# brownvc/matryodshka

Measured on AMD Instinct MI355X. Metric: novel-view frames/sec, 640x320 ODS->32-sphere MSI infer+render, higher is better.
Workload: dtype f32

## Files before the change

matryodshka_amd/csrc/cnn.hip:

```cpp
#include "cnn_plan.h"

namespace msi_cnn {

int device_cu_count() {
  int dev = 0;
  hipDeviceProp_t prop;
  if (hipGetDevice(&dev) != hipSuccess || hipGetDeviceProperties(&prop, dev) != hipSuccess || prop.multiProcessorCount <= 0) {
    (void)hipGetLastError();
    return DEFAULT_CUS;
  }
  return prop.multiProcessorCount;
}

int launch_conv(const LayerLaunch &Q, const ConvParams &p, hipStream_t stream) {
  const ConvVariant &V = Q.variant;
  int rc;
  switch (V.family) {
    case CONV_IGEMM: rc = launch_igemm(Q, p, stream); break;
    case CONV_HALO: case CONV_HALO_S2: case CONVT_HALO: rc = launch_halo_f32(Q, p, stream); break;
    case CONV_HALO_X3: case CONV_HALO8_X3: case CONV_HALO_S2_X3: case CONV_HALO8_S2_X3: case CONVT_HALO_X3: case CONVT_HALO8_X3: rc = launch_x3(Q, p, stream); break;
    case CONV_HALO_BF16: case CONV_HALO_BF16_S2: case CONVT_HALO_BF16: rc = launch_bf16_halo(Q, p, stream); break;
    default: return msi::fail(MSI_E_UNSUPPORTED, "conv: unknown kernel family %d", V.family);
  }
  if (rc || Q.nfix == 0 || p.tile_cnt != nullptr) return rc;
  const int mode = V.family == CONV_IGEMM ? V.mode : (V.is_convt() ? MODE_CONVT : MODE_CONV);
  return launch_fixup(V.bm, V.bn, mode, V.family == CONV_IGEMM && V.bf16 && mode != MODE_HEAD, Q.nfix, V.is_convt() ? 2 : 1, p, stream);
}

}

#if defined(MSI_CONV_TIMING) || defined(MSI_DEBUG_STATS)
static unsigned long long *g_timing_buf = nullptr;
static int g_timing_layer = -1;
extern "C" int msi_debug_conv_occupancy(int lds_bytes) {
  return msi_cnn::debug_conv_occupancy(lds_bytes);
}
extern "C" void msi_debug_conv_timing(void *device_buffer, int layer) {
  g_timing_buf = static_cast<unsigned long long *>(device_buffer);
  g_timing_layer = layer;
}
#endif

extern "C" {

#ifdef MSI_DEBUG_SUMS
extern "C" long long msi_debug_sums_offset(const msi_net_plan *plan, int layer) { return (long long)plan->net.layers[layer].sums_off; }
extern "C" long long msi_debug_partial_offset(const msi_net_plan *plan) { return (long long)plan->net.partial_off; }
#endif
static int run_layers(const msi_net_plan *plan, const float *packed, const void *net_input, float *pred,
                      void *workspace, size_t workspace_bytes, msi_stream_t stream_, int nlayers) {
  MSI_REQUIRE(plan, "net_forward: null plan");
  const msi_net_desc *desc = &plan->desc;
  const Net &net = plan->net;
  const int bf16 = desc->dtype == MSI_DTYPE_BF16;
  MSI_REQUIRE(packed && net_input && workspace, "net_forward: null pointer");
  if (workspace_bytes < net.ws_bytes)
    return msi::fail(MSI_E_WORKSPACE, "net_forward: workspace %zu B < required %zu B", workspace_bytes,
                     net.ws_bytes);
  if (desc->batch == 0) return MSI_OK;
  hipStream_t stream = msi::as_stream(stream_);
  char *ws = static_cast<char *>(workspace);
  {
    const size_t n16 = net.zero_bytes / 16;
    int rc0 = launch_zero(ws + net.zero_off, n16, stream);
    if (rc0) return rc0;
  }
  int *cnt = reinterpret_cast<int *>(ws + net.cnt_off);
  for (int li = 0; li < nlayers; ++li) {
    const Layer &L = net.layers[li];
    const LayerLaunch &Q = plan->launch[li];
    ConvParams p = Q.p;
    auto src_ptr = [&](int s) -> const char * {
      if (s < 0) return static_cast<const char *>(net_input);
      return ws + (bf16 ? net.layers[s].act_off : net.layers[s].raw_off);
    };
    p.x0 = src_ptr(L.src0);
    p.x1 = L.src1 >= 0 ? src_ptr(L.src1) : p.x0;
    p.wpk = reinterpret_cast<const char *>(packed + L.packed_off);
    p.coord_bias = L.has_coord ? packed + L.coord_off : nullptr;
    p.bias = L.kind == MODE_HEAD ? packed + L.gamma_off : nullptr;
    if (Q.fuse_ln) {
      const Layer &S = net.layers[L.src0];
      p.ln_sums = reinterpret_cast<const long long *>(ws + S.sums_off);
      p.ln_gamma = packed + S.gamma_off;
      p.ln_beta = packed + S.beta_off;
    }
    p.y = L.kind == MODE_HEAD ? pred : reinterpret_cast<float *>(ws + L.raw_off);
    p.sums = L.kind == MODE_HEAD ? nullptr : reinterpret_cast<long long *>(ws + L.sums_off);
    auto scl_of = [&](int li2) { return reinterpret_cast<const double *>(packed + net.layers[li2].lnscl_off); };
    p.ln_scl = L.kind == MODE_HEAD ? nullptr : scl_of(li);
    p.ln_scl_src = L.src0 >= 0 ? scl_of(L.src0) : nullptr;
    p.ln_scl_src1 = L.src1 >= 0 ? scl_of(L.src1) : nullptr;
    p.status = reinterpret_cast<int *>(ws + net.err_off);
    p.partial = reinterpret_cast<float *>(ws + net.partial_off);
// ... 139 lines not shown
  const Net &net = plan->net;
  const Layer &H = net.layers[MSI_NET_NUM_LAYERS - 1];
  const int nd = desc->num_outputs / 2;
  const int bf16 = desc->dtype == MSI_DTYPE_BF16;
  if ((!bf16 && !plan->launch[MSI_NET_NUM_LAYERS - 1].fuse_ln) || (bf16 && !plan->opt[MSI_NET_OPT_HEAD_FUSE_LN]) ||
      H.c0 > 64 || H.c0 % 4 != 0 || desc->num_outputs != 2 * nd || nd % 4 != 0 || nd > 64 || desc->in_channels != 6 * nd ||
      ((long)desc->height * desc->width) % HA_TP != 0)
    return msi::fail(MSI_E_UNSUPPORTED, "%s: fused tail needs a blend_psv network (in = 6 D, out = 2 D, "
                     "D %% 4 == 0, D <= 64, ngf <= 64, HEAD_FUSE_LN on)", who);
  MSI_REQUIRE(rgba_native || layers_out, "%s: null pointer", who);
  MSI_REQUIRE(!layers_out || (reinterpret_cast<uintptr_t>(layers_out) & 15) == 0, "%s: layers_out is not 16-byte aligned", who);
  const int ng = (nd + HA_LG - 1) / HA_LG;
  if (nd % ng != 0 || (nd / ng) % 4 != 0 || (ng > 1 && bf16 && (nd / ng) % 8 != 0))
    return msi::fail(MSI_E_UNSUPPORTED, "%s: D = %d does not split into layer groups of a multiple of %d", who, nd, bf16 ? 8 : 4);
  int rc = run_layers(plan, packed, net_input, nullptr, workspace, workspace_bytes, stream_, MSI_NET_NUM_LAYERS - 1);
  if (rc || desc->batch == 0) return rc;
  hipStream_t stream = msi::as_stream(stream_);
  if (event_after_convs) {
    hipError_t e = hipEventRecord(static_cast<hipEvent_t>(event_after_convs), stream);
    if (e != hipSuccess) return msi::fail(MSI_E_LAUNCH, "%s: %s", who, hipGetErrorString(e));
  }
  char *ws = static_cast<char *>(workspace);
  const Layer &S = net.layers[H.src0];
  HeadAsmParams q;
  q.x = reinterpret_cast<const float *>(ws + S.raw_off);
  q.wpk = packed + H.packed_off;
  q.bias = packed + H.gamma_off;
  float *aff = reinterpret_cast<float *>(ws + S.aff_off);
  rc = launch_ln_finish(desc->batch, stream, reinterpret_cast<const long long *>(ws + S.sums_off), 1.0 / S.ln_count,
                        reinterpret_cast<const double *>(packed + S.lnscl_off), reinterpret_cast<int *>(ws + net.err_off),
                        packed + S.gamma_off, packed + S.beta_off, S.cout, aff, bf16);
  if (rc) return rc;
  q.aff = aff;
  q.psv = net_input;
  q.rgba = reinterpret_cast<float4 *>(rgba_native);
  q.layers = layers_out;
  q.bw_out = blend_weights;
  q.al_out = alphas;
  q.pred_out = pred;
  q.C0 = H.c0; q.ksteps = H.ksteps; q.npad = H.npad;
  q.nd = nd; q.hw = desc->height * desc->width;
  q.npix_total = (long)desc->batch * q.hw;
  q.lg = nd / ng;
  q.ng = ng;
  {
    auto magic = [](unsigned d) { return d == 1 ? 0xffffffffu : (unsigned)((1ull << 32) / d); };
    const int vec = bf16 ? 8 : 4;
    const unsigned vpp = (unsigned)((ng == 1 ? 6 * nd : 2 * 3 * q.lg) / vec);
    q.mg_vpp = magic(vpp);
    q.mg_nchunk = magic((unsigned)(q.ksteps * 8));
    q.mg_hw = magic((unsigned)q.hw);
    if (q.npix_total >= (1L << 32)) return msi::fail(MSI_E_UNSUPPORTED, "%s: more than 2^32 pixels per batch", who);
  }
  constexpr int BN = 64;
  size_t r_bytes = (size_t)q.ksteps * (HA_TP + BN) * ROW_BYTES;
  if (r_bytes < (size_t)HA_TP * (6 * q.lg + 1) * sizeof(float)) r_bytes = (size_t)HA_TP * (6 * q.lg + 1) * sizeof(float);
  if (bf16) {
    r_bytes = (size_t)q.ksteps * HA_TP * ROW_BYTES;
    if (r_bytes < (size_t)HA_TP * (3 * q.lg + 1) * sizeof(unsigned)) r_bytes = (size_t)HA_TP * (3 * q.lg + 1) * sizeof(unsigned);
  }
  const size_t lds = 2 * 64 * 4 + 64 + ((r_bytes + 15) & ~(size_t)15) + (size_t)HA_TP * (2 * q.lg + 1) * sizeof(float);
  const long ntile = q.npix_total / HA_TP;
  if (((ntile + 7) / 8) * 8 * ng >= (1L << 31)) return msi::fail(MSI_E_UNSUPPORTED, "%s: too many pixel tiles for one launch", who);
  return launch_head_assemble(bf16, layers_out ? format : MSI_LAYERS_F32, (unsigned)(((ntile + 7) / 8) * 8 * ng), lds, stream, q);
}

int msi_net_plan_forward_rgba(const msi_net_plan *plan, const float *packed, const void *net_input, float *rgba_native,
                              float *blend_weights, float *alphas, float *pred, void *workspace, size_t workspace_bytes,
                              msi_stream_t stream_, void *event_after_convs) {
  return forward_fused_tail("net_forward_rgba", plan, packed, net_input, rgba_native, nullptr, MSI_LAYERS_F32, blend_weights, alphas, pred,
                            workspace, workspace_bytes, stream_, event_after_convs);
}

int msi_net_plan_forward_layers(const msi_net_plan *plan, const float *packed, const void *net_input, float *rgba_native,
                                void *layers_out, int32_t format, float *blend_weights, float *alphas, float *pred, void *workspace,
                                size_t workspace_bytes, msi_stream_t stream_, void *event_after_convs) {
  MSI_REQUIRE(!layers_out || format == MSI_LAYERS_RGBA8 || format == MSI_LAYERS_RGBA16F,
              "net_forward_layers: unknown format %d (layers_out is MSI_LAYERS_RGBA8 or MSI_LAYERS_RGBA16F)", format);
  MSI_REQUIRE(rgba_native || layers_out, "net_forward_layers: null pointer");
  return forward_fused_tail("net_forward_layers", plan, packed, net_input, rgba_native, layers_out, format, blend_weights, alphas, pred,
                            workspace, workspace_bytes, stream_, event_after_convs);
}

size_t msi_net_workspace_bytes(const msi_net_desc *desc) {
  msi_net_plan *pl = nullptr;
  if (msi_net_plan_create(desc, &pl)) return 0;
  const size_t n = pl->net.ws_bytes;
  msi_net_plan_destroy(pl);
  return n;
}

static int forward_once(const msi_net_desc *desc, const float *packed, const void *net_input, float *pred,
                        void *workspace, size_t workspace_bytes, msi_stream_t stream) {
  msi_net_plan *pl = nullptr;
  int rc = msi_net_plan_create(desc, &pl);
  if (rc) return rc;
  rc = msi_net_plan_forward(pl, packed, net_input, pred, workspace, workspace_bytes, stream);
  msi_net_plan_destroy(pl);
  return rc;
}

int msi_net_forward_f32(const msi_net_desc *desc, const float *packed, const float *net_input,
                        float *pred, void *workspace, size_t workspace_bytes, msi_stream_t stream) {
  MSI_REQUIRE(desc && desc->dtype == MSI_DTYPE_F32, "net_forward_f32: desc->dtype must be MSI_DTYPE_F32");
  return forward_once(desc, packed, net_input, pred, workspace, workspace_bytes, stream);
}

int msi_net_forward_bf16(const msi_net_desc *desc, const float *packed, const void *net_input_bf16,
                         float *pred, void *workspace, size_t workspace_bytes, msi_stream_t stream) {
  MSI_REQUIRE(desc && desc->dtype == MSI_DTYPE_BF16, "net_forward_bf16: desc->dtype must be MSI_DTYPE_BF16");
  return forward_once(desc, packed, net_input_bf16, pred, workspace, workspace_bytes, stream);
}

}
```

matryodshka_amd/csrc/cnn_device.h:

```cpp
#pragma once
#include <cmath>
#include <cstdint>
#include <cstdio>
#include <cstdlib>
#include <cstring>
#include <new>
#include <type_traits>
#include <vector>

#include "msi_common.h"

namespace msi_cnn {


typedef float f32x16 __attribute__((ext_vector_type(16)));
typedef float v4f __attribute__((ext_vector_type(4)));
typedef __attribute__((address_space(3))) void lds_void;

constexpr int BK = 32;
constexpr int ROW_BYTES = BK * 4;
#ifndef MSI_NSTAGE
#define MSI_NSTAGE 2
#endif
constexpr int NSTAGE = MSI_NSTAGE;
// ... 67 lines not shown
  int apply;
  int planes;
  int waves;
  bool is_halo() const { return family != CONV_IGEMM; }
  bool is_convt_f32() const { return family == CONVT_HALO || family == CONVT_HALO_X3 || family == CONVT_HALO8_X3; }
  bool is_convt() const { return is_convt_f32() || family == CONVT_HALO_BF16; }
  bool six_product() const { return family >= CONV_HALO_X3 && family <= CONVT_HALO8_X3; }
  bool tile8() const { return family == CONV_HALO8_X3 || family == CONV_HALO8_S2_X3 || family == CONVT_HALO8_X3; }
};

struct LayerLaunch {
  ConvParams p;
  ConvVariant variant;
  int nblocks, nfix;
  int inlaunch;
  int fuse_ln;
  int skip_apply;
  unsigned ln_blocks;
};

constexpr int HA_TP = 32;
#ifndef MSI_HA_LG
#define MSI_HA_LG 32
#endif
constexpr int HA_LG = MSI_HA_LG;

struct HeadAsmParams {
  const float *x;
  const float *wpk;
  const float *bias;
  const float *aff;
  const void *psv;
  float4 *rgba;
  float *bw_out, *al_out;
  float *pred_out;
  int C0, ksteps, npad, nd, hw;
  int lg, ng;
  unsigned mg_vpp, mg_nchunk, mg_hw;
  long npix_total;
  void *layers;
};

int launch_conv(const LayerLaunch &Q, const ConvParams &p, hipStream_t stream);
int launch_igemm(const LayerLaunch &Q, const ConvParams &p, hipStream_t stream);
int launch_fixup(int bm, int bn, int mode, int raw16, unsigned grid_x, unsigned grid_y, const ConvParams &p, hipStream_t stream);
int launch_halo_f32(const LayerLaunch &Q, const ConvParams &p, hipStream_t stream);
int launch_x3(const LayerLaunch &Q, const ConvParams &p, hipStream_t stream);
int launch_bf16_halo(const LayerLaunch &Q, const ConvParams &p, hipStream_t stream);
int launch_zero(void *p, size_t n16, hipStream_t stream);
int launch_ln_finish(int batch, hipStream_t stream, const long long *sums, double inv_n, const double *scl, int *status, const float *gamma, const float *beta, int C,
                     float *aff, int raw16);
int launch_ln_apply(int bf16out, unsigned blocks, int batch, size_t lds, hipStream_t stream, float *x, const long long *sums, double inv_n, const double *scl, int *status,
                    const float *gamma, const float *beta, size_t per_sample, int C, float *aff, unsigned short *yb);
int launch_head_assemble(int bf16in, int format, unsigned grid_x, size_t lds, hipStream_t stream, const HeadAsmParams &q);
int debug_conv_occupancy(int lds_bytes);

constexpr int vkey(int family, int a = 0, int b = 0, int c = 0, int d = 0, int e = 0) { return ((((family * 16 + a) * 16 + b) * 16 + c) * 16 + d) * 16 + e; }

inline int set_max_lds(const void *fn, int lds, unsigned long long &done, const char *what) {
  int dev = 0;
  if (hipGetDevice(&dev) != hipSuccess) dev = 0;
  const bool tracked = dev >= 0 && dev < 64;
  if (tracked && ((done >> dev) & 1ull)) return MSI_OK;
  hipError_t e = hipFuncSetAttribute(fn, hipFuncAttributeMaxDynamicSharedMemorySize, lds);
  if (e != hipSuccess) return msi::fail(MSI_E_LAUNCH, "%s: %s", what, hipGetErrorString(e));
  if (tracked) done |= 1ull << dev;
  return MSI_OK;
}

template <auto KERNEL, int LDS, int THREADS = 256>
int launch_kernel(unsigned nblocks, const ConvParams &p, hipStream_t stream, const char *what) {
  if constexpr (LDS > 65536) {
    static thread_local unsigned long long done = 0;
    int rc0 = set_max_lds(reinterpret_cast<const void *>(KERNEL), LDS, done, what);
    if (rc0) return rc0;
  }
  hipLaunchKernelGGL(KERNEL, dim3(nblocks), dim3(THREADS), LDS, stream, p);
  return msi::check_launch(what);
}

template <int N> using IC = std::integral_constant<int, N>;
}
using namespace msi_cnn;

namespace {

template <int MODE>
__device__ __forceinline__ int tap_delta(int v, int parity, int rate, bool wrapt) {
  if (MODE == MODE_CONV) return v * rate;
  if (MODE == MODE_CONVT) return wrapt ? -v : (v == 0 ? 0 : (parity ? 1 : -1));
  return 0;
}

__device__ __forceinline__ unsigned udiv_magic(unsigned x, unsigned d, unsigned mg) {
  unsigned q = __umulhi(x, mg);
  if (x - q * d >= d) ++q;
  return q;
}

__device__ __forceinline__ int halo_row(const ConvParams &p, int tyi, int r, int rows_per_tile) {
  return p.row_par ? (tyi >> 1) * (2 * rows_per_tile) + (tyi & 1) + 2 * r : tyi * rows_per_tile + r;
}

__device__ __forceinline__ int xcd_contiguous(int bid, int n) {
  const int q = n >> 3, r = n & 7, xcd = bid & 7, local = bid >> 3;
  return (xcd < r ? xcd * (q + 1) : r * (q + 1) + (xcd - r) * q) + local;
}
// ... 618 lines not shown
```

matryodshka_amd/csrc/cnn_tail.hip:

```cpp
#include "cnn_device.h"

namespace {


template <int BF16IN>
__global__ void __launch_bounds__(256) __attribute__((amdgpu_waves_per_eu(BF16IN ? 6 : 5)))
head_assemble_kernel(const HeadAsmParams p) {
  [[maybe_unused]] constexpr int FMT = MSI_LAYERS_F32;
#include "cnn_tail_head_assemble.inc"
}

template <int BF16IN, int FMT>
__global__ void __launch_bounds__(256) __attribute__((amdgpu_waves_per_eu(BF16IN ? 6 : 5)))
head_assemble_packed_kernel(const HeadAsmParams p) {
  static_assert(FMT == MSI_LAYERS_RGBA8 || FMT == MSI_LAYERS_RGBA16F, "a packed texel format");
#include "cnn_tail_head_assemble.inc"
}

__global__ void __launch_bounds__(256)
ln_finish_kernel(const long long *__restrict__ sums, double inv_n, const double *__restrict__ scl, int *status,
                 const float *__restrict__ gamma, const float *__restrict__ beta, int C, float *__restrict__ aff, int raw16) {
  __shared__ double s_stat[2];
  const int b = blockIdx.x, tid = threadIdx.x;
  ln_mean_inv(sums + (size_t)b * LN_SHARDS * LN_WORDS, inv_n, scl, status, s_stat, tid);
  const double mu = s_stat[0], inv = s_stat[1];
  const double up = raw16 ? scl[2] * 16777216.0 : 1.0;
  for (int c = tid; c < C; c += 256) {
    const double sc = inv * (double)gamma[c];
    aff[(size_t)b * 2 * C + c] = (float)(sc * up);
    aff[(size_t)b * 2 * C + C + c] = (float)((double)beta[c] - mu * sc);
  }
}

__global__ void __launch_bounds__(256) zero_kernel(float4 *__restrict__ p, size_t n16) {
  const size_t i = (size_t)blockIdx.x * 256 + threadIdx.x;
  if (i < n16) p[i] = float4{0.f, 0.f, 0.f, 0.f};
}

template <int BF16OUT>
__global__ void __launch_bounds__(256)
ln_apply_kernel(float *__restrict__ x, const long long *__restrict__ sums, double inv_n, const double *__restrict__ scl,
                int *status, const float *__restrict__ gamma, const float *__restrict__ beta, size_t per_sample, int C,
                float *__restrict__ aff, unsigned short *__restrict__ yb) {
  extern __shared__ __attribute__((aligned(16))) float s_aff[];
  __shared__ double s_stat[2];
  const int b = blockIdx.y, tid = threadIdx.x;
  ln_mean_inv(sums + (size_t)b * LN_SHARDS * LN_WORDS, inv_n, scl, (blockIdx.x == 0 ? status : nullptr), s_stat, tid);
  const double mu = s_stat[0], inv = s_stat[1];
  const double up = BF16OUT ? scl[2] * 16777216.0 : 1.0;
  for (int c = tid; c < C; c += 256) {
    const double sc = inv * (double)gamma[c];
    const float fs = (float)sc, ft = (float)((double)beta[c] - mu * sc);
    s_aff[c] = BF16OUT ? (float)(sc * up) : fs;
    s_aff[C + c] = ft;
    if (blockIdx.x == 0) {
      aff[(size_t)b * 2 * C + c] = fs;
      aff[(size_t)b * 2 * C + C + c] = ft;
    }
  }
  __syncthreads();

  typedef _Float16 h4_t __attribute__((ext_vector_type(4)));
  const h4_t *xh = reinterpret_cast<const h4_t *>(reinterpret_cast<const _Float16 *>(x) + (size_t)b * per_sample);
  v4f *xv = reinterpret_cast<v4f *>(x + (size_t)b * per_sample);
  auto get = [&](size_t i) __attribute__((always_inline)) -> v4f {
    if (BF16OUT == 1) { const h4_t h = xh[i]; return v4f{(float)h.x, (float)h.y, (float)h.z, (float)h.w}; }
    return xv[i];
  };
  const size_t nvec = per_sample / 4;
  const size_t stride = (size_t)gridDim.x * blockDim.x;
  auto apply = [](v4f v, const v4f s4, const v4f t4) __attribute__((always_inline)) -> v4f {
    v.x = fmaxf(v.x * s4.x + t4.x, 0.f);
    v.y = fmaxf(v.y * s4.y + t4.y, 0.f);
    v.z = fmaxf(v.z * s4.z + t4.z, 0.f);
    v.w = fmaxf(v.w * s4.w + t4.w, 0.f);
    return v;
  };
  auto bf16_bits = [](float f) __attribute__((always_inline)) -> unsigned {
    const unsigned u = __builtin_bit_cast(unsigned, f);
    return (u + 0x7fffu + ((u >> 16) & 1u)) >> 16;
  };
  typedef unsigned v2u __attribute__((ext_vector_type(2)));
  v2u *yv = reinterpret_cast<v2u *>(yb + (size_t)b * per_sample);
  auto put = [&](size_t i, const v4f v) __attribute__((always_inline)) {
    if (BF16OUT == 1) yv[i] = v2u{bf16_bits(v.x) | (bf16_bits(v.y) << 16), bf16_bits(v.z) | (bf16_bits(v.w) << 16)};
    else xv[i] = v;
  };
  if ((256 * 4) % C == 0) {
    const int c = (tid * 4) % C;
    const v4f s4 = *reinterpret_cast<const v4f *>(s_aff + c);
    const v4f t4 = *reinterpret_cast<const v4f *>(s_aff + C + c);
    for (size_t i = (size_t)blockIdx.x * blockDim.x + tid; i < nvec; i += stride) put(i, apply(get(i), s4, t4));
  } else {
    for (size_t i = (size_t)blockIdx.x * blockDim.x + tid; i < nvec; i += stride) {
      const int c = (int)((i * 4) % C);
      put(i, apply(get(i), *reinterpret_cast<const v4f *>(s_aff + c), *reinterpret_cast<const v4f *>(s_aff + C + c)));
    }
  }
}

}

namespace msi_cnn {
int launch_zero(void *ptr, size_t n16, hipStream_t stream) {
  hipLaunchKernelGGL(zero_kernel, dim3((unsigned)((n16 + 255) / 256)), dim3(256), 0, stream, reinterpret_cast<float4 *>(ptr), n16);
  return msi::check_launch("zero");
}
int launch_ln_finish(int batch, hipStream_t stream, const long long *sums, double inv_n, const double *scl, int *status, const float *gamma, const float *beta, int C,
                     float *aff, int raw16) {
  hipLaunchKernelGGL(ln_finish_kernel, dim3(batch), dim3(256), 0, stream, sums, inv_n, scl, status, gamma, beta, C, aff, raw16);
  return msi::check_launch("ln_finish");
}
int launch_ln_apply(int bf16out, unsigned blocks, int batch, size_t lds, hipStream_t stream, float *x, const long long *sums, double inv_n, const double *scl, int *status,
                    const float *gamma, const float *beta, size_t per_sample, int C, float *aff, unsigned short *yb) {
  const dim3 grid(blocks, batch);
  if (bf16out) hipLaunchKernelGGL(ln_apply_kernel<1>, grid, dim3(256), lds, stream, x, sums, inv_n, scl, status, gamma, beta, per_sample, C, aff, yb);
  else hipLaunchKernelGGL(ln_apply_kernel<0>, grid, dim3(256), lds, stream, x, sums, inv_n, scl, status, gamma, beta, per_sample, C, aff, yb);
  return msi::check_launch("ln_apply");
}
int launch_head_assemble(int bf16in, int format, unsigned grid_x, size_t lds, hipStream_t stream, const HeadAsmParams &q) {
#define MSI_LAUNCH_HA(K) hipLaunchKernelGGL(K, dim3(grid_x), dim3(256), lds, stream, q)
  switch (format) {
    case MSI_LAYERS_F32:
      if (bf16in) MSI_LAUNCH_HA(head_assemble_kernel<1>); else MSI_LAUNCH_HA(head_assemble_kernel<0>);
      break;
    case MSI_LAYERS_RGBA8:
      if (bf16in) MSI_LAUNCH_HA((head_assemble_packed_kernel<1, MSI_LAYERS_RGBA8>)); else MSI_LAUNCH_HA((head_assemble_packed_kernel<0, MSI_LAYERS_RGBA8>));
      break;
    case MSI_LAYERS_RGBA16F:
      if (bf16in) MSI_LAUNCH_HA((head_assemble_packed_kernel<1, MSI_LAYERS_RGBA16F>)); else MSI_LAUNCH_HA((head_assemble_packed_kernel<0, MSI_LAYERS_RGBA16F>));
      break;
    default:
      return msi::fail(MSI_E_BADARG, "head_assemble: unknown format %d", format);
  }
#undef MSI_LAUNCH_HA
  return msi::check_launch("head_assemble");
}
}
```

matryodshka_amd/csrc/cnn_tail_head_assemble.inc:

```
#if defined(__HIP_DEVICE_COMPILE__)
  extern __shared__ __attribute__((aligned(16))) char smem[];
  constexpr int BN = 64;
  const int tid = threadIdx.x, lane = tid & 63, wave = tid >> 6;
  const int nd = p.nd, lg = p.lg, ng = p.ng;
  const unsigned slot = blockIdx.x >> 3;
  const unsigned tsl = ng == 1 ? slot : (ng == 2 ? slot >> 1 : slot / (unsigned)ng);
  const int g = (int)(slot - tsl * (unsigned)ng);
  const long tile = (long)tsl * 8 + (blockIdx.x & 7u);
  if (tile * HA_TP >= p.npix_total) return;
  const int c_psv = 6 * nd, c_pred = 2 * nd;
  const int l_cpsv = 6 * lg, l_cpred = 2 * lg;
  const int s_psv = l_cpsv + 1, s_pred = l_cpred + 1;
  const int s_psv16 = 3 * lg + 1;
  float *s_aff = reinterpret_cast<float *>(smem);
  char *sR = smem + 2 * 64 * 4 + 64;
  char *sA = sR;
  char *sB = sA + p.ksteps * HA_TP * ROW_BYTES;
  const size_t r_bytes = BF16IN ? max((size_t)p.ksteps * HA_TP * ROW_BYTES, (size_t)HA_TP * s_psv16 * sizeof(unsigned))
                                : max((size_t)p.ksteps * (HA_TP + BN) * ROW_BYTES, (size_t)HA_TP * s_psv * sizeof(float));
  float *l_psv = reinterpret_cast<float *>(sR);
  float *l_pred = reinterpret_cast<float *>(sR + ((r_bytes + 15) & ~(size_t)15));
  auto gcol = [&](int n) __attribute__((always_inline)) -> int { return n < lg ? g * lg + n : nd + g * lg + (n - lg); };

  const long p0 = tile * HA_TP;
  const int b = (int)udiv_magic((unsigned)p0, (unsigned)p.hw, p.mg_hw);
  constexpr int PSV_PER_THREAD = BF16IN ? 3 : 6;
  constexpr int B_PER_THREAD = 4;
  constexpr int PSV_VEC = BF16IN ? 8 : 4;
  constexpr int ESZ = BF16IN ? 2 : 4;
  const int nrun = ng == 1 ? 1 : 2;
  const int run_len = ng == 1 ? c_psv : 3 * lg;
  const int vpr = run_len / PSV_VEC, vpp = nrun * vpr;
  const int nv_psv = HA_TP * vpp;
  float4 q[PSV_PER_THREAD];
  {
    const char *gp = static_cast<const char *>(p.psv) + (size_t)p0 * c_psv * ESZ;
#pragma unroll
    for (int k = 0; k < PSV_PER_THREAD; ++k) {
      const int v = tid + 256 * k;
      if (v < nv_psv) {
        if (ng == 1) {
          q[k] = reinterpret_cast<const float4 *>(gp)[v];
        } else {
          const int px = (int)udiv_magic((unsigned)v, (unsigned)vpp, p.mg_vpp), w = v - px * vpp;
          const int r = w >= vpr ? 1 : 0, idx = w - r * vpr;
          const int start = r == 0 ? 3 * g * lg : 3 * (nd + g * lg);
          q[k] = *reinterpret_cast<const float4 *>(gp + ((size_t)px * c_psv + start + idx * PSV_VEC) * ESZ);
        }
      }
    }
  }
  const int nchunk = p.ksteps * 8;
  v4f araw[2];
  if (BF16IN) {
    typedef _Float16 h8_t __attribute__((ext_vector_type(8)));
    const int r = tid >> 3, c = (tid & 7) * 8;
    araw[0] = araw[1] = v4f{0.f, 0.f, 0.f, 0.f};
    if (c < p.C0) {
      const h8_t h = *reinterpret_cast<const h8_t *>(reinterpret_cast<const _Float16 *>(p.x) + (size_t)(p0 + r) * p.C0 + c);
      araw[0] = v4f{(float)h[0], (float)h[1], (float)h[2], (float)h[3]};
      araw[1] = v4f{(float)h[4], (float)h[5], (float)h[6], (float)h[7]};
    }
  } else {
#pragma unroll
    for (int k = 0; k < 2; ++k) {
      const int e = tid + 256 * k;
      const int r = (int)udiv_magic((unsigned)e, (unsigned)nchunk, p.mg_nchunk), c = (e - r * nchunk) * 4;
      araw[k] = v4f{0.f, 0.f, 0.f, 0.f};
      if (e < HA_TP * nchunk && c < p.C0) araw[k] = *reinterpret_cast<const v4f *>(p.x + (size_t)(p0 + r) * p.C0 + c);
    }
  }
  const int nb = p.ksteps * BN * 8;
  v4f braw[B_PER_THREAD];
  v4f wfrag[4];
  if (BF16IN) {
    if (wave < 2) {
      const int frow = lane & 31, fh = lane >> 5;
      const int nloc = wave * 32 + frow;
      const int gn = gcol(nloc < l_cpred ? nloc : 0);
      const int fswz = (gn >> 1) & 7;
#pragma unroll
      for (int qq = 0; qq < 4; ++qq) {
        wfrag[qq] = v4f{0.f, 0.f, 0.f, 0.f};
        if (nloc < l_cpred)
          wfrag[qq] = *reinterpret_cast<const v4f *>(p.wpk + (size_t)gn * (ROW_BYTES / 4) + (((2 * qq + fh) ^ fswz) << 2));
      }
    }
  } else {
#pragma unroll
    for (int k = 0; k < B_PER_THREAD; ++k) {
      const int e = tid + 256 * k;
      const int row = e >> 3, j = e & 7;
      const int ks = row / BN, n = row - ks * BN;
      braw[k] = v4f{0.f, 0.f, 0.f, 0.f};
      if (e < nb && n < l_cpred)
        braw[k] = *reinterpret_cast<const v4f *>(p.wpk + ((size_t)ks * p.npad + gcol(n)) * (ROW_BYTES / 4) + j * 4);
    }
  }
  if (tid < 2 * p.C0) s_aff[tid] = p.aff[(size_t)b * 2 * p.C0 + tid];
  __syncthreads();
  if (BF16IN) {
    const int r = tid >> 3, ch = tid & 7, c = ch * 8;
    unsigned pk[4] = {0u, 0u, 0u, 0u};
    if (c < p.C0) {
      float y[8];
#pragma unroll
      for (int k = 0; k < 2; ++k) {
        const v4f s4 = *reinterpret_cast<const v4f *>(s_aff + c + 4 * k), t4 = *reinterpret_cast<const v4f *>(s_aff + p.C0 + c + 4 * k);
        y[4 * k] = fmaxf(araw[k].x * s4.x + t4.x, 0.f); y[4 * k + 1] = fmaxf(araw[k].y * s4.y + t4.y, 0.f);
        y[4 * k + 2] = fmaxf(araw[k].z * s4.z + t4.z, 0.f); y[4 * k + 3] = fmaxf(araw[k].w * s4.w + t4.w, 0.f);
      }
#pragma unroll
      for (int k = 0; k < 4; ++k) asm("v_cvt_pk_bf16_f32 %0, %1, %2" : "=v"(pk[k]) : "v"(y[2 * k]), "v"(y[2 * k + 1]));
    }
    typedef unsigned v4u_t __attribute__((ext_vector_type(4)));
    *reinterpret_cast<v4u_t *>(sA + r * ROW_BYTES + ((ch ^ ((r >> 1) & 7)) << 4)) = v4u_t{pk[0], pk[1], pk[2], pk[3]};
  } else
#pragma unroll
  for (int k = 0; k < 2; ++k) {
    const int e = tid + 256 * k;
    if (e < HA_TP * nchunk) {
      const int r = (int)udiv_magic((unsigned)e, (unsigned)nchunk, p.mg_nchunk), ch = e - r * nchunk;
      const int c = ch * 4;
      v4f y = {0.f, 0.f, 0.f, 0.f};
      if (c < p.C0) {
        const v4f s4 = *reinterpret_cast<const v4f *>(s_aff + c), t4 = *reinterpret_cast<const v4f *>(s_aff + p.C0 + c);
        y.x = fmaxf(araw[k].x * s4.x + t4.x, 0.f); y.y = fmaxf(araw[k].y * s4.y + t4.y, 0.f);
        y.z = fmaxf(araw[k].z * s4.z + t4.z, 0.f); y.w = fmaxf(araw[k].w * s4.w + t4.w, 0.f);
      }
      const int ks = ch >> 3, chunk = ch & 7;
      *reinterpret_cast<v4f *>(sA + (ks * HA_TP + r) * ROW_BYTES + ((chunk ^ ((r >> 1) & 7)) << 4)) = y;
    }
  }
  if (!BF16IN) {
#pragma unroll
    for (int k = 0; k < B_PER_THREAD; ++k) {
      const int e = tid + 256 * k;
      if (e < nb) *reinterpret_cast<v4f *>(sB + (e >> 3) * ROW_BYTES + ((e & 7) << 4)) = braw[k];
    }
  }
  __syncthreads();
  if (wave < 2) {
    f32x16 acc;
#pragma unroll
    for (int r = 0; r < 16; ++r) acc[r] = 0.f;
    const int frow = lane & 31, fh = lane >> 5;
    const int fswz_a = (frow >> 1) & 7;
    const int fswz_b = (gcol(wave * 32 + frow < l_cpred ? wave * 32 + frow : 0) >> 1) & 7;
    if (BF16IN) {
      typedef __bf16 bf16x8 __attribute__((ext_vector_type(8)));
#pragma unroll
      for (int qq = 0; qq < 4; ++qq) {
        const v4f a = *reinterpret_cast<const v4f *>(sA + frow * ROW_BYTES + (((2 * qq + fh) ^ fswz_a) << 4));
        acc = __builtin_amdgcn_mfma_f32_32x32x16_bf16(__builtin_bit_cast(bf16x8, wfrag[qq]), __builtin_bit_cast(bf16x8, a), acc, 0, 0, 0);
      }
    } else
    for (int ks = 0; ks < p.ksteps; ++ks) {
#pragma unroll
      for (int qq = 0; qq < 4; ++qq) {
        const v4f a = *reinterpret_cast<const v4f *>(sA + (ks * HA_TP + frow) * ROW_BYTES + (((fh * 4 + qq) ^ fswz_a) << 4));
        const v4f w = *reinterpret_cast<const v4f *>(sB + (ks * BN + wave * 32 + frow) * ROW_BYTES + (((fh * 4 + qq) ^ fswz_b) << 4));
        acc = __builtin_amdgcn_mfma_f32_32x32x2f32(w.x, a.x, acc, 0, 0, 0);
        acc = __builtin_amdgcn_mfma_f32_32x32x2f32(w.y, a.y, acc, 0, 0, 0);
        acc = __builtin_amdgcn_mfma_f32_32x32x2f32(w.z, a.z, acc, 0, 0, 0);
        acc = __builtin_amdgcn_mfma_f32_32x32x2f32(w.w, a.w, acc, 0, 0, 0);
      }
    }
    const int px = lane & 31, half = lane >> 5;
#pragma unroll
    for (int gg = 0; gg < 4; ++gg) {
      const int n = wave * 32 + 8 * gg + 4 * half;
      if (n < l_cpred) {
        const int gn = gcol(n);
        const v4f bs = *reinterpret_cast<const v4f *>(p.bias + gn);
        v4f t = {msi_tanh(acc[4 * gg] + bs.x), msi_tanh(acc[4 * gg + 1] + bs.y), msi_tanh(acc[4 * gg + 2] + bs.z), msi_tanh(acc[4 * gg + 3] + bs.w)};
        if (p.pred_out) *reinterpret_cast<v4f *>(p.pred_out + (p0 + px) * c_pred + gn) = t;
        t.x = (t.x + 1.0f) / 2.0f; t.y = (t.y + 1.0f) / 2.0f; t.z = (t.z + 1.0f) / 2.0f; t.w = (t.w + 1.0f) / 2.0f;
        float *dst = l_pred + px * s_pred + n;
        dst[0] = t.x; dst[1] = t.y; dst[2] = t.z; dst[3] = t.w;
        if (n < lg) {
          if (p.bw_out) *reinterpret_cast<v4f *>(p.bw_out + (p0 + px) * nd + gn) = t;
        } else {
          if (p.al_out) *reinterpret_cast<v4f *>(p.al_out + (p0 + px) * nd + (gn - nd)) = t;
        }
      }
    }
  }
  __syncthreads();
#pragma unroll
  for (int k = 0; k < PSV_PER_THREAD; ++k) {
    const int v = tid + 256 * k;
    if (v < nv_psv) {
      const int px = (int)udiv_magic((unsigned)v, (unsigned)vpp, p.mg_vpp), w = v - px * vpp;
      if (BF16IN) {
        unsigned *dst = reinterpret_cast<unsigned *>(l_psv) + px * s_psv16 + w * 4;
        dst[0] = __builtin_bit_cast(unsigned, q[k].x); dst[1] = __builtin_bit_cast(unsigned, q[k].y);
        dst[2] = __builtin_bit_cast(unsigned, q[k].z); dst[3] = __builtin_bit_cast(unsigned, q[k].w);
      } else {
        float *dst = l_psv + px * s_psv + w * PSV_VEC;
        dst[0] = q[k].x; dst[1] = q[k].y; dst[2] = q[k].z; dst[3] = q[k].w;
      }
    }
  }
  __syncthreads();
  {
#pragma clang fp contract(off)
    const int px = tid & (HA_TP - 1);
    const long pp = p0 + px;
    const long off = pp - (long)b * p.hw;
    const float *rp = l_psv + px * s_psv;
    const float *rq = l_pred + px * s_pred;
    float4 *dst = p.rgba + ((long)b * nd + g * lg + tid / HA_TP) * p.hw + off;
    const long dstep = (long)(256 / HA_TP) * p.hw;
    constexpr int TEXEL_BYTES = FMT == MSI_LAYERS_RGBA8 ? 4 : 8;
    char *dstp = FMT != MSI_LAYERS_F32 ? static_cast<char *>(p.layers) + (((long)b * nd + g * lg + tid / HA_TP) * p.hw + off) * TEXEL_BYTES : nullptr;
    const bool want_f32 = FMT == MSI_LAYERS_F32 || p.rgba != nullptr;
    const unsigned *rp16 = reinterpret_cast<const unsigned *>(l_psv) + px * s_psv16;
    for (int d = tid / HA_TP; d < lg; d += 256 / HA_TP, dst += dstep, dstp += dstep * TEXEL_BYTES) {
      float fgv[3], bgv[3];
      if (BF16IN) {
        const int ef = 3 * d, eb = 3 * (lg + d);
        const unsigned f0 = rp16[ef >> 1], f1 = rp16[(ef >> 1) + 1], b0 = rp16[eb >> 1], b1 = rp16[(eb >> 1) + 1];
        const unsigned long long fw = ((unsigned long long)f1 << 32 | f0) >> ((ef & 1) * 16), bw = ((unsigned long long)b1 << 32 | b0) >> ((eb & 1) * 16);
#pragma unroll
        for (int c = 0; c < 3; ++c) {
          fgv[c] = __builtin_bit_cast(float, (unsigned)(fw >> (16 * c)) << 16);
          bgv[c] = __builtin_bit_cast(float, (unsigned)(bw >> (16 * c)) << 16);
        }
      } else {
#pragma unroll
        for (int c = 0; c < 3; ++c) { fgv[c] = rp[d * 3 + c]; bgv[c] = rp[(lg + d) * 3 + c]; }
      }
      const float *fg = fgv;
      const float *bg = bgv;
      const float w = rq[d];
      const float omw = 1.0f - w;
      float4 o;
      o.x = w * fg[0] + omw * bg[0];
      o.y = w * fg[1] + omw * bg[1];
      o.z = w * fg[2] + omw * bg[2];
      o.w = rq[lg + d];
      if constexpr (FMT == MSI_LAYERS_RGBA8) *reinterpret_cast<unsigned *>(dstp) = rgba8_encode(o);
      else if constexpr (FMT == MSI_LAYERS_RGBA16F) *reinterpret_cast<u32x2_g *>(dstp) = rgba16f_encode(o);
      if (want_f32) {
#if defined(MSI_HA_NT) && MSI_HA_NT
        __builtin_nontemporal_store(o.x, &dst->x); __builtin_nontemporal_store(o.y, &dst->y); __builtin_nontemporal_store(o.z, &dst->z); __builtin_nontemporal_store(o.w, &dst->w);
#else
        *dst = o;
#endif
      }
    }
  }
#endif
```

matryodshka_amd/isa_lint.py:

```python
import os
import re
import struct
import subprocess
import sys
import tempfile

def _find_objdump():
    import shutil
    cands = [os.environ.get("LLVM_OBJDUMP")]
    hipcc = os.environ.get("HIPCC") or shutil.which("hipcc") or "/opt/rocm/bin/hipcc"
    if hipcc and os.path.exists(hipcc):
        root = os.path.dirname(os.path.dirname(os.path.realpath(hipcc)))
        cands += [os.path.join(root, "lib", "llvm", "bin", "llvm-objdump"), os.path.join(root, "llvm", "bin", "llvm-objdump")]
    cands += [os.path.join(os.environ.get("ROCM_PATH", "/opt/rocm"), "lib", "llvm", "bin", "llvm-objdump"), "/opt/rocm/lib/llvm/bin/llvm-objdump",
              shutil.which("llvm-objdump")]
    for c in cands:
        if c and os.path.exists(c):
            return c
    raise RuntimeError("isa_lint: llvm-objdump not found (set LLVM_OBJDUMP)")


OBJDUMP = None
MAGIC = b"__CLANG_OFFLOAD_BUNDLE__"
FORBIDDEN = re.compile(r"^\s*(v_pk_(?:mul|add|fma)_f32|v_pk_mov_b32)\b.*\bop_sel:\[[01,]*1[01,]*\]")
# ... 16 lines not shown
        return None
    ops = [o.strip() for o in m.group(2).split(",")]
    data = ops[0] if "buffer" in m.group(1) else (ops[1] if len(ops) > 1 else "")
    return _vrange(data)


def _valu_dest(ins):
    t = ins.strip()
    if not t.startswith("v_") or t.startswith(NOT_A_VGPR_WRITE):
        return None
    parts = t.split(None, 1)
    if len(parts) < 2:
        return None
    return _vrange(parts[1].split(",")[0])


LOAD = re.compile(r"^(?:t?buffer_load_|global_load_|flat_load_|scratch_load_|ds_read|ds_load|ds_bpermute|ds_permute|ds_swizzle|ds_consume|ds_append|image_)")
DS_RETURN = re.compile(r"^ds_\w+_rtn_")
ATOMIC_RETURN = re.compile(r"^(?:buffer|global|flat)_atomic_")


def vgpr_writes(ins):
    t = ins.strip()
    parts = t.split(None, 1)
    if len(parts) < 2:
        return []
    mn, ops = parts[0], [o.strip() for o in parts[1].split(",")]
    out = []
    if mn.startswith("v_"):
        d = _valu_dest(t)
        if d is not None:
            out.append((d, "valu"))
        if mn.startswith("v_swap_b32") and len(ops) > 1 and _vrange(ops[1].split()[0]) is not None:
            out.append((_vrange(ops[1].split()[0]), "valu"))
    elif LOAD.match(mn) or DS_RETURN.match(mn):
        if re.search(r"\blds\b", parts[1]):
            return []
        d = _vrange(ops[0].split()[0]) if ops and ops[0] else None
        if d is not None:
            out.append((d, "load"))
    elif ATOMIC_RETURN.match(mn) and re.search(r"\b(?:glc|sc0)\b", parts[1]):
        d = _vrange(ops[0].split()[0]) if ops and ops[0] else None
        if d is not None:
            out.append((d, "load"))
    return out


def scan_kernel_text(lines):
    bad = []
    nstore = nload = 0
    pending = []
    for ins in lines:
        if not ins.strip():
            continue
        if pending:
            writes = vgpr_writes(ins)
            keep = []
            for p in pending:
                hit = [k for d, k in writes if not (d[1] < p[0][0] or d[0] > p[0][1])]
                if hit and "valu" not in hit:
                    nload += 1
                if "valu" in hit:
                    bad.append(p[1] + "  -> (%d wait state(s)) ->  " % p[2] + ins.strip())
                    continue
                mn = re.match(r"\s*s_nop\s+(\d+)", ins)
                p[2] += int(mn.group(1)) + 1 if mn else 1
                if p[2] < WIDE_STORE_WAIT_STATES:
                    keep.append(p)
            pending = keep
        sd = _store_data(ins)
        if sd is not None:
            nstore += 1
            pending.append([sd, ins.strip(), 0])
    return bad, nstore, nload


def _fatbin_section(path):
    data = open(path, "rb").read()
    assert data[:4] == b"\x7fELF" and data[4] == 2, "64-bit ELF expected"
    shoff, = struct.unpack_from("<Q", data, 0x28)
    shentsize, shnum, shstrndx = struct.unpack_from("<HHH", data, 0x3A)
    def sh(i):
        name, typ, flags, addr, off, size = struct.unpack_from("<IIQQQQ", data, shoff + i * shentsize)
        return name, off, size
    _, stroff, strsize = sh(shstrndx)
    for i in range(shnum):
        name, off, size = sh(i)
        end = data.index(b"\0", stroff + name)
        if data[stroff + name:end] == b".hip_fatbin":
            return data[off:off + size]
    raise RuntimeError("no .hip_fatbin section in " + path)


def code_objects(path):
    sec = _fatbin_section(path)
    out = []
    pos = sec.find(MAGIC)
    while pos >= 0:
        n, = struct.unpack_from("<Q", sec, pos + len(MAGIC))
        p = pos + len(MAGIC) + 8
        for _ in range(n):
            off, size, tlen = struct.unpack_from("<QQQ", sec, p)
            triple = sec[p + 24:p + 24 + tlen].decode()
            p += 24 + tlen
            if "amdgcn" in triple and size:
                out.append((triple, sec[pos + off:pos + off + size]))
# ... 50 lines not shown
```

Measured before the change: 539.2.

## Add direct head-assemble path reading sweep volume into registers, skipping LDS staging

Adds a DIRECT variant of the fused head-assemble kernel for the fp32 path. Each thread loads its pixel's foreground and background PSV colors straight from global memory into registers. It computes the blend in registers and writes the RGBA texels directly, so the LDS staging of the sweep volume and the B-operand LDS buffer go away. The MFMA uses fp32 32x32x2 on register weight fragments, and the second k-step's weights can be loaded late. The aim is smaller LDS use, which allows more waves per EU, plus fewer barriers. The cost is wider strided global reads and writes that coalesce less well, and a slower fp32 MFMA form.

```diff
diff --git a/matryodshka_amd/csrc/cnn.hip b/matryodshka_amd/csrc/cnn.hip
--- a/matryodshka_amd/csrc/cnn.hip
+++ b/matryodshka_amd/csrc/cnn.hip
@@ -1,4 +1,6 @@
 #include "cnn_plan.h"
+
+#include <atomic>
 
 namespace msi_cnn {
 
@@ -40,6 +42,10 @@
   g_timing_layer = layer;
 }
 #endif
+
+static std::atomic<int> g_tail_form{-1};
+static int tail_form_default(int out_format) { return out_format == MSI_LAYERS_F32 ? 0 : 1; }
+extern "C" int msi_debug_tail_form(int form) { return g_tail_form.exchange(form < 0 ? -1 : (form ? 1 : 0)); }
 
 extern "C" {
 
@@ -285,9 +291,13 @@
     q.mg_hw = magic((unsigned)q.hw);
     if (q.npix_total >= (1L << 32)) return msi::fail(MSI_E_UNSUPPORTED, "%s: more than 2^32 pixels per batch", who);
   }
+  const int out_format = layers_out ? format : MSI_LAYERS_F32;
+  const int forced = g_tail_form.load(std::memory_order_relaxed);
+  const int direct = bf16 ? 0 : (forced >= 0 ? forced : tail_form_default(out_format));
   constexpr int BN = 64;
   size_t r_bytes = (size_t)q.ksteps * (HA_TP + BN) * ROW_BYTES;
   if (r_bytes < (size_t)HA_TP * (6 * q.lg + 1) * sizeof(float)) r_bytes = (size_t)HA_TP * (6 * q.lg + 1) * sizeof(float);
+  if (direct) r_bytes = (size_t)q.ksteps * HA_TP * ROW_BYTES;
   if (bf16) {
     r_bytes = (size_t)q.ksteps * HA_TP * ROW_BYTES;
     if (r_bytes < (size_t)HA_TP * (3 * q.lg + 1) * sizeof(unsigned)) r_bytes = (size_t)HA_TP * (3 * q.lg + 1) * sizeof(unsigned);
@@ -295,7 +305,7 @@
   const size_t lds = 2 * 64 * 4 + 64 + ((r_bytes + 15) & ~(size_t)15) + (size_t)HA_TP * (2 * q.lg + 1) * sizeof(float);
   const long ntile = q.npix_total / HA_TP;
   if (((ntile + 7) / 8) * 8 * ng >= (1L << 31)) return msi::fail(MSI_E_UNSUPPORTED, "%s: too many pixel tiles for one launch", who);
-  return launch_head_assemble(bf16, layers_out ? format : MSI_LAYERS_F32, (unsigned)(((ntile + 7) / 8) * 8 * ng), lds, stream, q);
+  return launch_head_assemble(bf16, direct, out_format, (unsigned)(((ntile + 7) / 8) * 8 * ng), lds, stream, q);
 }
 
 int msi_net_plan_forward_rgba(const msi_net_plan *plan, const float *packed, const void *net_input, float *rgba_native,
diff --git a/matryodshka_amd/csrc/cnn_device.h b/matryodshka_amd/csrc/cnn_device.h
--- a/matryodshka_amd/csrc/cnn_device.h
+++ b/matryodshka_amd/csrc/cnn_device.h
@@ -143,7 +143,7 @@
                      float *aff, int raw16);
 int launch_ln_apply(int bf16out, unsigned blocks, int batch, size_t lds, hipStream_t stream, float *x, const long long *sums, double inv_n, const double *scl, int *status,
                     const float *gamma, const float *beta, size_t per_sample, int C, float *aff, unsigned short *yb);
-int launch_head_assemble(int bf16in, int format, unsigned grid_x, size_t lds, hipStream_t stream, const HeadAsmParams &q);
+int launch_head_assemble(int bf16in, int direct, int format, unsigned grid_x, size_t lds, hipStream_t stream, const HeadAsmParams &q);
 int debug_conv_occupancy(int lds_bytes);
 
 constexpr int vkey(int family, int a = 0, int b = 0, int c = 0, int d = 0, int e = 0) { return ((((family * 16 + a) * 16 + b) * 16 + c) * 16 + d) * 16 + e; }
diff --git a/matryodshka_amd/csrc/cnn_tail.hip b/matryodshka_amd/csrc/cnn_tail.hip
--- a/matryodshka_amd/csrc/cnn_tail.hip
+++ b/matryodshka_amd/csrc/cnn_tail.hip
@@ -1,4 +1,11 @@
 #include "cnn_device.h"
+
+#ifndef MSI_HA_DIRECT_WAVES
+#define MSI_HA_DIRECT_WAVES 6
+#endif
+#ifndef MSI_HA_DIRECT_WSPLIT
+#define MSI_HA_DIRECT_WSPLIT 1
+#endif
 
 namespace {
 
@@ -7,6 +14,7 @@
 __global__ void __launch_bounds__(256) __attribute__((amdgpu_waves_per_eu(BF16IN ? 6 : 5)))
 head_assemble_kernel(const HeadAsmParams p) {
   [[maybe_unused]] constexpr int FMT = MSI_LAYERS_F32;
+  [[maybe_unused]] constexpr bool DIRECT = false;
 #include "cnn_tail_head_assemble.inc"
 }
 
@@ -14,6 +22,23 @@
 __global__ void __launch_bounds__(256) __attribute__((amdgpu_waves_per_eu(BF16IN ? 6 : 5)))
 head_assemble_packed_kernel(const HeadAsmParams p) {
   static_assert(FMT == MSI_LAYERS_RGBA8 || FMT == MSI_LAYERS_RGBA16F, "a packed texel format");
+  [[maybe_unused]] constexpr bool DIRECT = false;
+#include "cnn_tail_head_assemble.inc"
+}
+
+__global__ void __launch_bounds__(256) __attribute__((amdgpu_waves_per_eu(MSI_HA_DIRECT_WAVES)))
+head_assemble_direct_kernel(const HeadAsmParams p) {
+  [[maybe_unused]] constexpr int BF16IN = 0, FMT = MSI_LAYERS_F32;
+  [[maybe_unused]] constexpr bool DIRECT = true;
+#include "cnn_tail_head_assemble.inc"
+}
+
+template <int FMT>
+__global__ void __launch_bounds__(256) __attribute__((amdgpu_waves_per_eu(MSI_HA_DIRECT_WAVES)))
+head_assemble_direct_packed_kernel(const HeadAsmParams p) {
+  static_assert(FMT == MSI_LAYERS_RGBA8 || FMT == MSI_LAYERS_RGBA16F, "a packed texel format");
+  [[maybe_unused]] constexpr int BF16IN = 0;
+  [[maybe_unused]] constexpr bool DIRECT = true;
 #include "cnn_tail_head_assemble.inc"
 }
 
@@ -118,8 +143,18 @@
   else hipLaunchKernelGGL(ln_apply_kernel<0>, grid, dim3(256), lds, stream, x, sums, inv_n, scl, status, gamma, beta, per_sample, C, aff, yb);
   return msi::check_launch("ln_apply");
 }
-int launch_head_assemble(int bf16in, int format, unsigned grid_x, size_t lds, hipStream_t stream, const HeadAsmParams &q) {
+int launch_head_assemble(int bf16in, int direct, int format, unsigned grid_x, size_t lds, hipStream_t stream, const HeadAsmParams &q) {
 #define MSI_LAUNCH_HA(K) hipLaunchKernelGGL(K, dim3(grid_x), dim3(256), lds, stream, q)
+  if (direct && bf16in) return msi::fail(MSI_E_UNSUPPORTED, "head_assemble: the direct form reads an fp32 sweep volume");
+  if (direct) {
+    switch (format) {
+      case MSI_LAYERS_F32: MSI_LAUNCH_HA(head_assemble_direct_kernel); break;
+      case MSI_LAYERS_RGBA8: MSI_LAUNCH_HA(head_assemble_direct_packed_kernel<MSI_LAYERS_RGBA8>); break;
+      case MSI_LAYERS_RGBA16F: MSI_LAUNCH_HA(head_assemble_direct_packed_kernel<MSI_LAYERS_RGBA16F>); break;
+      default: return msi::fail(MSI_E_BADARG, "head_assemble: unknown format %d", format);
+    }
+    return msi::check_launch("head_assemble");
+  }
   switch (format) {
     case MSI_LAYERS_F32:
       if (bf16in) MSI_LAUNCH_HA(head_assemble_kernel<1>); else MSI_LAUNCH_HA(head_assemble_kernel<0>);
diff --git a/matryodshka_amd/csrc/cnn_tail_head_assemble.inc b/matryodshka_amd/csrc/cnn_tail_head_assemble.inc
--- a/matryodshka_amd/csrc/cnn_tail_head_assemble.inc
+++ b/matryodshka_amd/csrc/cnn_tail_head_assemble.inc
@@ -12,11 +12,15 @@
   const int l_cpsv = 6 * lg, l_cpred = 2 * lg;
   const int s_psv = l_cpsv + 1, s_pred = l_cpred + 1;
   const int s_psv16 = 3 * lg + 1;
+  static_assert(!DIRECT || !BF16IN, "the direct form reads an fp32 sweep volume");
+  const int dpx = tid >> 3, dj = tid & 7;
+  const bool d_owns = 4 * dj < lg;
   float *s_aff = reinterpret_cast<float *>(smem);
   char *sR = smem + 2 * 64 * 4 + 64;
   char *sA = sR;
   char *sB = sA + p.ksteps * HA_TP * ROW_BYTES;
-  const size_t r_bytes = BF16IN ? max((size_t)p.ksteps * HA_TP * ROW_BYTES, (size_t)HA_TP * s_psv16 * sizeof(unsigned))
+  const size_t r_bytes = DIRECT ? (size_t)p.ksteps * HA_TP * ROW_BYTES
+                       : BF16IN ? max((size_t)p.ksteps * HA_TP * ROW_BYTES, (size_t)HA_TP * s_psv16 * sizeof(unsigned))
                                 : max((size_t)p.ksteps * (HA_TP + BN) * ROW_BYTES, (size_t)HA_TP * s_psv * sizeof(float));
   float *l_psv = reinterpret_cast<float *>(sR);
   float *l_pred = reinterpret_cast<float *>(sR + ((r_bytes + 15) & ~(size_t)15));
@@ -33,7 +37,14 @@
   const int vpr = run_len / PSV_VEC, vpp = nrun * vpr;
   const int nv_psv = HA_TP * vpp;
   float4 q[PSV_PER_THREAD];
-  {
+  if (DIRECT) {
+    if (d_owns) {
+      const float *rowp = static_cast<const float *>(p.psv) + (size_t)(p0 + dpx) * c_psv + 12 * dj;
+      const float4 *fgp = reinterpret_cast<const float4 *>(rowp + 3 * g * lg), *bgp = reinterpret_cast<const float4 *>(rowp + 3 * (nd + g * lg));
+#pragma unroll
+      for (int k = 0; k < 3; ++k) { q[k] = fgp[k]; q[3 + k] = bgp[k]; }
+    }
+  } else {
     const char *gp = static_cast<const char *>(p.psv) + (size_t)p0 * c_psv * ESZ;
 #pragma unroll
     for (int k = 0; k < PSV_PER_THREAD; ++k) {
@@ -72,8 +83,25 @@
   }
   const int nb = p.ksteps * BN * 8;
   v4f braw[B_PER_THREAD];
-  v4f wfrag[4];
-  if (BF16IN) {
+  v4f wfrag[DIRECT ? 8 : 4];
+  auto load_wfrag = [&](int ks) __attribute__((always_inline)) {
+    const int frow = lane & 31, fh = lane >> 5;
+    const int nloc = wave * 32 + frow;
+    const int gn = gcol(nloc < l_cpred ? nloc : 0);
+    const int fswz = (gn >> 1) & 7;
+#pragma unroll
+    for (int qq = 0; qq < 4; ++qq) {
+      wfrag[4 * ks + qq] = v4f{0.f, 0.f, 0.f, 0.f};
+      if (ks < p.ksteps && nloc < l_cpred)
+        wfrag[4 * ks + qq] = *reinterpret_cast<const v4f *>(p.wpk + ((size_t)ks * p.npad + gn) * (ROW_BYTES / 4) + (((fh * 4 + qq) ^ fswz) << 2));
+    }
+  };
+  if (DIRECT) {
+    if (wave < 2) {
+#pragma unroll
+      for (int ks = 0; ks < (MSI_HA_DIRECT_WSPLIT ? 1 : 2); ++ks) load_wfrag(ks);
+    }
+  } else if (BF16IN) {
     if (wave < 2) {
       const int frow = lane & 31, fh = lane >> 5;
       const int nloc = wave * 32 + frow;
@@ -132,7 +160,7 @@
       *reinterpret_cast<v4f *>(sA + (ks * HA_TP + r) * ROW_BYTES + ((chunk ^ ((r >> 1) & 7)) << 4)) = y;
     }
   }
-  if (!BF16IN) {
+  if (!BF16IN && !DIRECT) {
 #pragma unroll
     for (int k = 0; k < B_PER_THREAD; ++k) {
       const int e = tid + 256 * k;
@@ -153,6 +181,22 @@
       for (int qq = 0; qq < 4; ++qq) {
         const v4f a = *reinterpret_cast<const v4f *>(sA + frow * ROW_BYTES + (((2 * qq + fh) ^ fswz_a) << 4));
         acc = __builtin_amdgcn_mfma_f32_32x32x16_bf16(__builtin_bit_cast(bf16x8, wfrag[qq]), __builtin_bit_cast(bf16x8, a), acc, 0, 0, 0);
+      }
+    } else if (DIRECT) {
+#pragma unroll
+      for (int ks = 0; ks < 2; ++ks) {
+        if (ks < p.ksteps) {
+          if (MSI_HA_DIRECT_WSPLIT && ks == 1) load_wfrag(1);
+#pragma unroll
+          for (int qq = 0; qq < 4; ++qq) {
+            const v4f a = *reinterpret_cast<const v4f *>(sA + (ks * HA_TP + frow) * ROW_BYTES + (((fh * 4 + qq) ^ fswz_a) << 4));
+            const v4f w = wfrag[4 * ks + qq];
+            acc = __builtin_amdgcn_mfma_f32_32x32x2f32(w.x, a.x, acc, 0, 0, 0);
+            acc = __builtin_amdgcn_mfma_f32_32x32x2f32(w.y, a.y, acc, 0, 0, 0);
+            acc = __builtin_amdgcn_mfma_f32_32x32x2f32(w.z, a.z, acc, 0, 0, 0);
+            acc = __builtin_amdgcn_mfma_f32_32x32x2f32(w.w, a.w, acc, 0, 0, 0);
+          }
+        }
       }
     } else
     for (int ks = 0; ks < p.ksteps; ++ks) {
@@ -187,6 +231,7 @@
     }
   }
   __syncthreads();
+  if (!DIRECT) {
 #pragma unroll
   for (int k = 0; k < PSV_PER_THREAD; ++k) {
     const int v = tid + 256 * k;
@@ -203,7 +248,40 @@
     }
   }
   __syncthreads();
-  {
+  }
+  if (DIRECT) {
+#pragma clang fp contract(off)
+    if (d_owns) {
+      const long off = p0 + dpx - (long)b * p.hw;
+      const float *rq = l_pred + dpx * s_pred + 4 * dj;
+      const long texel = ((long)b * nd + g * lg + 4 * dj) * p.hw + off;
+      float4 *dst = p.rgba + texel;
+      constexpr int TEXEL_BYTES = FMT == MSI_LAYERS_RGBA8 ? 4 : 8;
+      char *dstp = FMT != MSI_LAYERS_F32 ? static_cast<char *>(p.layers) + texel * TEXEL_BYTES : nullptr;
+      const bool want_f32 = FMT == MSI_LAYERS_F32 || p.rgba != nullptr;
+      const float fg[12] = {q[0].x, q[0].y, q[0].z, q[0].w, q[1].x, q[1].y, q[1].z, q[1].w, q[2].x, q[2].y, q[2].z, q[2].w};
+      const float bg[12] = {q[3].x, q[3].y, q[3].z, q[3].w, q[4].x, q[4].y, q[4].z, q[4].w, q[5].x, q[5].y, q[5].z, q[5].w};
+#pragma unroll
+      for (int i = 0; i < 4; ++i, dst += p.hw, dstp += (long)p.hw * TEXEL_BYTES) {
+        const float w = rq[i];
+        const float omw = 1.0f - w;
+        float4 o;
+        o.x = w * fg[3 * i] + omw * bg[3 * i];
+        o.y = w * fg[3 * i + 1] + omw * bg[3 * i + 1];
+        o.z = w * fg[3 * i + 2] + omw * bg[3 * i + 2];
+        o.w = rq[lg + i];
+        if constexpr (FMT == MSI_LAYERS_RGBA8) *reinterpret_cast<unsigned *>(dstp) = rgba8_encode(o);
+        else if constexpr (FMT == MSI_LAYERS_RGBA16F) *reinterpret_cast<u32x2_g *>(dstp) = rgba16f_encode(o);
+        if (want_f32) {
+#if defined(MSI_HA_NT) && MSI_HA_NT
+          __builtin_nontemporal_store(o.x, &dst->x); __builtin_nontemporal_store(o.y, &dst->y); __builtin_nontemporal_store(o.z, &dst->z); __builtin_nontemporal_store(o.w, &dst->w);
+#else
+          *dst = o;
+#endif
+        }
+      }
+    }
+  } else {
 #pragma clang fp contract(off)
     const int px = tid & (HA_TP - 1);
     const long pp = p0 + px;
diff --git a/matryodshka_amd/isa_lint.py b/matryodshka_amd/isa_lint.py
--- a/matryodshka_amd/isa_lint.py
+++ b/matryodshka_amd/isa_lint.py
@@ -92,6 +92,9 @@
     pending = []
     for ins in lines:
         if not ins.strip():
+            continue
+        if re.match(r"\s*s_endpgm\b", ins):
+            pending = []
             continue
         if pending:
             writes = vgpr_writes(ins)
```

New measurement: 537.5. No clear change (-0.3%).
